# 10XGenomics/lariat

Measured on AMD Instinct MI355X. Metric: read-pairs/sec aligned to hg38 (per-barcode align loop: SMEM seeding + SW + RFA/MAPQ on device); synthetic hg38-scale reference, higher is better.
Workload: dtype u64/i32 (FM-index + integer DP), f64 (RFA scores)

## Files before the change

### lariat_amd/csrc/k_chain_lane.h

```cpp
#pragma once
#include "k_extend2.h"

#ifndef LH_CHAIN_LANE_WAVES
#define LH_CHAIN_LANE_WAVES 2
#endif
#define LH_CHAIN_LANE_MAXC 8
#define CLW(ci_, f_) cl[(((ci_) << 3) + (f_)) * 64 + lane]
#define NIB(x_, i_) ((int)(((x_) >> ((i_) << 2)) & 0xf))
#define NIB_SET(x_, i_, v_) ((x_) = ((x_) & ~(0xfu << ((i_) << 2))) | ((uint32_t)(v_) << ((i_) << 2)))
template <class Lt> __device__ __forceinline__ void dev_introsort_small_nib(int n, uint32_t& a, Lt lt, int32_t* wdp) {
    if (n < 1) return;
    if (n == 2) {
        if (lt(NIB(a, 1), NIB(a, 0))) { int x = NIB(a, 0), y = NIB(a, 1); NIB_SET(a, 0, y); NIB_SET(a, 1, x); }
        return;
    }
    if (n > 1) {
        int t = n - 1, i = 0, j = t, k = i + ((j - i) >> 1) + 1;
        if (lt(NIB(a, k), NIB(a, i))) {
            if (lt(NIB(a, k), NIB(a, j))) k = j;
        } else k = lt(NIB(a, j), NIB(a, i)) ? i : j;
        const int rp = NIB(a, k);
        if (k != t) { int y = NIB(a, t); NIB_SET(a, k, y); NIB_SET(a, t, rp); }
        int wd = 4 * LH_CHAIN_LANE_MAX + 8;
        for (;;) {
            do { ++i; LH_WATCH(wdp, wd, 4, return) } while (lt(NIB(a, i), rp));
            do { --j; LH_WATCH(wdp, wd, 5, return) } while (i <= j && lt(rp, NIB(a, j)));
            if (j <= i) break;
            int x = NIB(a, i), y = NIB(a, j); NIB_SET(a, i, y); NIB_SET(a, j, x);
        }
        { int x = NIB(a, i), y = NIB(a, t); NIB_SET(a, i, y); NIB_SET(a, t, x); }
    }
    for (int i = 1; i < n; ++i)
        for (int j = i; j > 0 && lt(NIB(a, j), NIB(a, j - 1)); --j) { int x = NIB(a, j), y = NIB(a, j - 1); NIB_SET(a, j, y); NIB_SET(a, j - 1, x); }
}
__global__ void __launch_bounds__(64, LH_CHAIN_LANE_WAVES) k_chain_lane(DIndex ix, DOpts o, int n_reads, i64 pool_cap, const DSeed* __restrict__ seeds, const int32_t* __restrict__ s_rid,
                                                    const int32_t* __restrict__ l_rep, DChain* __restrict__ chains, DSeed* __restrict__ cseeds, int32_t* __restrict__ n_chains,
                                                    int32_t* __restrict__ status, int32_t* __restrict__ list, int32_t* __restrict__ list_count, int32_t* __restrict__ srt,
                                                    i64* __restrict__ chain_rmax, DCounters* __restrict__ ctr, ExtArgs A, int fuse,
                                                    int32_t* __restrict__ next_count, int32_t* __restrict__ next_list, int32_t* __restrict__ next_key,
                                                    int32_t* __restrict__ defer_count, int32_t* __restrict__ defer_list) {
    const i64* __restrict__ seq_off = A.seq_off; const i64* __restrict__ seed_off = A.seed_off; int32_t* __restrict__ sdone = A.sdone;
    __shared__ uint32_t cl[LH_CHAIN_LANE_MAXC * 8 * 64];
    const int r = blockIdx.x * blockDim.x + threadIdx.x, lane = LANE();
    int heavy = 0, ext_out = 0, ext_key = 0;
    u64 win = 0, cells = 0;
    int nch_done = 0;
    if (r < n_reads) {
        const i64 base = seed_off[r];
        const int S = (int)(seed_off[r + 1] - base);
        if (seed_off[r + 1] > pool_cap) { n_chains[r] = 0; A.n_regs[r] = 0; atomicOr(&status[r], LH_ST_POOL_OVERFLOW); }
        else if (S > LH_CHAIN_LANE_MAX) heavy = 1;
        else {
            const int len = (int)(seq_off[r + 1] - seq_off[r]);
            const DSeed* sd_ = seeds + base;
            const int32_t* rid_ = s_rid + base;
            int nch = 0;
            uint32_t od = 0;
            u64 smap0 = ~0ull, smap1 = ~0ull;
#define SMAP_SET(s_, v_) { if ((s_) < 16) smap0 = (smap0 & ~(0xfull << ((s_) << 2))) | ((u64)(v_) << ((s_) << 2)); else smap1 = (smap1 & ~(0xfull << (((s_) - 16) << 2))) | ((u64)(v_) << (((s_) - 16) << 2)); }
#define SMAP_GET(s_) ((int)((((s_) < 16 ? smap0 : smap1) >> (((s_) & 15) << 2)) & 0xf))
            DSeed pn; pn.rbeg = 0; pn.qbeg = 0; pn.len = 0;
            int ridn = -1;
            if (S > 0) { pn = sd_[0]; ridn = rid_[0]; }
            for (int s = 0; s < S && !heavy; ++s) {
                const DSeed p = pn;
                const int rid = ridn;
                if (s + 1 < S) { pn = sd_[s + 1]; ridn = rid_[s + 1]; }
                if (rid < 0) continue;
                int to_add = 1, lo = 0;
                for (int k = 0; k < nch; ++k) {
                    const int ci = NIB(od, k);
                    const i64 pos = (i64)((u64)CLW(ci, 0) | (u64)CLW(ci, 1) << 32);
                    if (pos <= p.rbeg) lo = k + 1; else break;
                }
                if (lo > 0) {
                    const int ci = NIB(od, lo - 1);
                    const i64 c_pos = (i64)((u64)CLW(ci, 0) | (u64)CLW(ci, 1) << 32);
                    const uint32_t qp = CLW(ci, 3), ridw = CLW(ci, 4);
                    const i64 c_last_rbeg = c_pos + (int32_t)CLW(ci, 2);
                    const int c_first_qbeg = qp & 0xff, c_last_qbeg = (qp >> 8) & 0xff, c_last_len = (qp >> 16) & 0xff, c_rid = (int)(ridw & 0x3fffffffu);
                    const i64 qend = c_last_qbeg + c_last_len, rend = c_last_rbeg + c_last_len;
                    int res = 0;
                    if (rid != c_rid) res = 0;
                    else if (p.qbeg >= c_first_qbeg && p.qbeg + p.len <= qend && p.rbeg >= c_pos && p.rbeg + p.len <= rend) res = 1;
                    else if ((c_last_rbeg < ix.l_pac || c_pos < ix.l_pac) && p.rbeg >= ix.l_pac) res = 0;
                    else {
                        i64 x = p.qbeg - c_last_qbeg, y = p.rbeg - c_last_rbeg;
                        if (y >= 0 && x - y <= o.w && y - x <= o.w && x - c_last_len < o.max_chain_gap && y - c_last_len < o.max_chain_gap) res = 2;
                    }
                    if (res == 2) {
                        const int rr = (int)(p.rbeg - c_pos);
                        CLW(ci, 2) = (uint32_t)rr;
                        CLW(ci, 3) = (uint32_t)c_first_qbeg | (uint32_t)p.qbeg << 8 | (uint32_t)p.len << 16;
                        uint32_t w5 = CLW(ci, 5), w6 = CLW(ci, 6);
                        int n = w5 & 0xff, wq = (int)(w5 >> 8), endq = w6 & 0xff, wr = (int)(w6 >> 8), endr = (int32_t)CLW(ci, 7);
                        if (p.qbeg >= endq) wq += p.len; else if (p.qbeg + p.len > endq) wq += p.qbeg + p.len - endq;
                        endq = endq > p.qbeg + p.len ? endq : p.qbeg + p.len;
                        if (rr >= endr) wr += p.len; else if (rr + p.len > endr) wr += rr + p.len - endr;
                        endr = endr > rr + p.len ? endr : rr + p.len;
                        CLW(ci, 5) = (uint32_t)(n + 1) | (uint32_t)wq << 8; CLW(ci, 6) = (uint32_t)endq | (uint32_t)wr << 8; CLW(ci, 7) = (uint32_t)endr;
                        SMAP_SET(s, ci)
                    }
                    to_add = (res == 0);
                }
                if (to_add) {
                    if (nch == LH_CHAIN_LANE_MAXC) { heavy = 1; break; }
                    const uint32_t lowm = lo ? (0xffffffffu >> (32 - (lo << 2))) : 0u;
                    od = (od & lowm) | ((uint32_t)nch << (lo << 2)) | ((lo < 7) ? ((od & ~lowm) << 4) : 0u);
                    CLW(nch, 0) = (uint32_t)(u64)p.rbeg; CLW(nch, 1) = (uint32_t)((u64)p.rbeg >> 32); CLW(nch, 2) = 0;
                    CLW(nch, 3) = (uint32_t)p.qbeg | (uint32_t)p.qbeg << 8 | (uint32_t)p.len << 16;
                    CLW(nch, 4) = (uint32_t)rid | ((ix.contig_alt && ix.contig_alt[rid]) ? 1u << 30 : 0u);
                    CLW(nch, 5) = 1u | (uint32_t)p.len << 8; CLW(nch, 6) = (uint32_t)(p.qbeg + p.len) | (uint32_t)p.len << 8; CLW(nch, 7) = (uint32_t)p.len;
                    SMAP_SET(s, nch)
                    nch++;
                }
            }
            if (!heavy) {
            for (int k = 0; k < nch; ++k) {
                const uint32_t w5 = CLW(k, 5), w6 = CLW(k, 6);
                int wq = (int)(w5 >> 8), wr = (int)(w6 >> 8);
                int w = wr < wq ? wr : wq;
                CLW(k, 6) = (uint32_t)(w < 1 << 30 ? w : (1 << 30) - 1);
                CLW(k, 5) = w5 & 0xff;
            }
#define C_W(id_) ((int)CLW(id_, 6))
#define C_BEG(id_) ((int)(CLW(id_, 3) & 0xff))
#define C_END(id_) ((int)(((CLW(id_, 3) >> 8) & 0xff) + ((CLW(id_, 3) >> 16) & 0xff)))
#define C_KEPT(id_) ((int)((CLW(id_, 5) >> 8) & 0xff))
#define C_SET_KEPT(id_, v_) (CLW(id_, 5) = (CLW(id_, 5) & ~0xff00u) | ((uint32_t)(v_) << 8))
#define C_FIRST(id_) ((int)((CLW(id_, 5) >> 16) & 0xff) - 1)
#define C_SET_FIRST(id_, v_) (CLW(id_, 5) = (CLW(id_, 5) & ~0xff0000u) | ((uint32_t)((v_) + 1) << 16))
            uint32_t st = 0;
            int n = 0;
            for (int k = 0; k < nch; ++k) {
                const int id = NIB(od, k);
                if (C_W(id) < o.min_chain_weight) continue;
                NIB_SET(st, n, id); n++;
            }
            if (n > 0) {
                dev_introsort_small_nib(n, st, [&](int x, int y) { return C_W(x) > C_W(y); }, o.wd);
                uint32_t kl = 0;
                int nk = 0;
                C_SET_KEPT(NIB(st, 0), 3);
                NIB_SET(kl, nk, 0); nk++;
                for (int i = 1; i < n; ++i) {
                    int large_ovlp = 0, k;
                    const int idi = NIB(st, i);
                    const int ai_beg = C_BEG(idi), ai_end = C_END(idi), ai_w = C_W(idi), ai_alt = (int)(CLW(idi, 4) >> 30) & 1;
                    for (k = 0; k < nk; ++k) {
                        const int idj = NIB(st, NIB(kl, k));
                        const int aj_beg = C_BEG(idj), aj_end = C_END(idj), aj_w = C_W(idj), aj_alt = (int)(CLW(idj, 4) >> 30) & 1;
                        int b_max = aj_beg > ai_beg ? aj_beg : ai_beg;
                        int e_min = aj_end < ai_end ? aj_end : ai_end;
                        if (e_min > b_max && (!aj_alt || ai_alt)) {
                            int li = ai_end - ai_beg, lj = aj_end - aj_beg;
                            int min_l = li < lj ? li : lj;
                            if (e_min - b_max >= min_l * o.mask_level && min_l < o.max_chain_gap) {
                                large_ovlp = 1;
                                if (C_FIRST(idj) < 0) C_SET_FIRST(idj, i);
                                if (ai_w < aj_w * o.drop_ratio && aj_w - ai_w >= o.min_seed_len << 1) break;
                            }
                        }
                    }
                    if (k == nk) { NIB_SET(kl, nk, i); nk++; C_SET_KEPT(idi, large_ovlp ? 2 : 3); }
                }
                for (int i = 0; i < nk; ++i) {
                    int f = C_FIRST(NIB(st, NIB(kl, i)));
                    if (f >= 0) C_SET_KEPT(NIB(st, f), 1);
                }
                int i, k;
                for (i = k = 0; i < n; ++i) {
                    int kp = C_KEPT(NIB(st, i));
                    if (kp == 0 || kp == 3) continue;
                    if (++k >= o.max_chain_extend) break;
                }
                for (; i < n; ++i)
                    if (C_KEPT(NIB(st, i)) < 3) C_SET_KEPT(NIB(st, i), 0);
            }
            int m = 0, sstart = 0;
            const float frac_rep = (float)l_rep[r] / len;
            for (int i = 0; i < n; ++i) {
                const int id = NIB(st, i);
                const int kp = C_KEPT(id);
                if (kp == 0) { CLW(id, 7) = 0xffffffffu; continue; }
                DChain oc;
                oc.pos = (i64)((u64)CLW(id, 0) | (u64)CLW(id, 1) << 32); oc.rid = (int)(CLW(id, 4) & 0x3fffffffu); oc.n = (int)(CLW(id, 5) & 0xff); oc.seed_start = sstart;
                oc.w = C_W(id); oc.kept = kp; oc.is_alt = (int)(CLW(id, 4) >> 30) & 1;
                oc.frac_rep = frac_rep; oc.pad = id;
                chains[base + m] = oc;
                CLW(id, 7) = (uint32_t)sstart; CLW(id, 2) = 0;
                sstart += oc.n;
                m++;
            }
            for (int k = 0; k < nch; ++k) if (C_W(k) < o.min_chain_weight) CLW(k, 7) = 0xffffffffu;
            for (int s = 0; s < S; ++s) {
                const int id = SMAP_GET(s);
                if (id == 0xf) continue;
                const uint32_t ss = CLW(id, 7);
                if (ss == 0xffffffffu) continue;
                const uint32_t t = CLW(id, 2);
                cseeds[base + ss + t] = sd_[s];
                CLW(id, 2) = t + 1;
            }
            n_chains[r] = m;
#undef SMAP_SET
#undef SMAP_GET
#undef C_W
#undef C_BEG
#undef C_END
#undef C_KEPT
#undef C_SET_KEPT
#undef C_FIRST
#undef C_SET_FIRST
            {
                int l_query = len > LH_MAXLEN ? 0 : len;
                const i64 l_pac = ix.l_pac;
                for (int ci = 0; ci < m; ++ci) {
                    DChain c = chains[base + ci];
                    const DSeed* sd = cseeds + base + c.seed_start;
                    int32_t* so = srt + base + c.seed_start;
                    int32_t* done = sdone + base + c.seed_start;
                    const int n = c.n;
                    if (n == 0) continue;
                    i64 r0 = l_pac << 1, r1 = 0;
                    for (int i = 0; i < n; ++i) {
                        DSeed t = sd[i];
                        i64 b = t.rbeg - (t.qbeg + dev_cal_max_gap(o, t.qbeg));
                        i64 e = t.rbeg + t.len + ((l_query - t.qbeg - t.len) + dev_cal_max_gap(o, l_query - t.qbeg - t.len));
                        r0 = r0 < b ? r0 : b;
                        r1 = r1 > e ? r1 : e;
                    }
                    i64 rmax0 = r0 > 0 ? r0 : 0, rmax1 = r1 < l_pac << 1 ? r1 : l_pac << 1;
                    DSeed s0 = sd[0];
                    if (rmax0 < l_pac && l_pac < rmax1) {
                        if (s0.rbeg < l_pac) rmax1 = l_pac;
                        else rmax0 = l_pac;
                    }
                    dev_fetch_clamp(ix, &rmax0, s0.rbeg, &rmax1);
                    win += (u64)(rmax1 - rmax0);
                    chain_rmax[2 * (base + ci)] = rmax0; chain_rmax[2 * (base + ci) + 1] = rmax1;
                    for (int i = 0; i < n; ++i) {
                        DSeed t = sd[i];
                        int rank = 0;
                        for (int u = 0; u < n; ++u) { DSeed x = sd[u]; rank += (x.len < t.len) || (x.len == t.len && u < i); }
                        so[rank] = i;
                        done[i] = 1;
                    }
                }
                nch_done = m;
            }
            if (fuse) ext_out = ext_control<false>(ix, o, A, r, nullptr, lane, &ext_key, &cells);
            }
        }
    }
    ext_append(ext_out, r, ext_key, lane, next_count, next_list, next_key, defer_count, defer_list);
    if (ctr) {
        unsigned w32 = (unsigned)win;
        u64 wtot = (u64)(uint32_t)wave_sum_i32((int)(w32 >> 16)) << 16;
        wtot += (u64)(uint32_t)wave_sum_i32((int)(w32 & 0xffff));
        int ctot = wave_sum_i32(nch_done);
        if (lane == 0 && (wtot || ctot)) { atomicAdd(&LH_CTR(ctr)->win_bases, wtot); atomicAdd(&LH_CTR(ctr)->n_chain_ext, (u64)ctot); }
    }
    u64 hm = __ballot(heavy);
    if (hm) {
        int basep = 0;
        if (lane == 0) basep = atomicAdd(list_count, (int32_t)__popcll(hm));
        basep = wave_readlane(basep, 0);
        if (heavy) list[basep + lanes_below(hm, lane)] = r;
    }
}
```

### lariat_amd/csrc/k_extend2.h

```cpp
#pragma once
#include "k_extend.h"

#define EH_H(v) ((int)((v) & 0xffffu))
#define EH_E(v) ((int)(((v) >> 16) & 0x1fffu))
#define EH_Q(v) ((int)((v) >> 29))
#define EH_PACK(q, e, h) ((uint32_t)(q) << 29 | (uint32_t)(e) << 16 | (uint32_t)(h))

#define LH_EXT_CIRC_MAX_W 30
__device__ __forceinline__ ExtRes lane_ksw_extend2(const DOpts& o, const uint8_t* q, uint32_t* ehl, int lane, int qoff, int qstep, int qlen, LaneTgt& tg, int tlen, int w,
                                                   int end_bonus, int zdrop, int h0, u64* cells, int circ_mask) {
    const int a_ = o.a, b_ = o.b, o_del = o.o_del, e_del = o.e_del, o_ins = o.o_ins, e_ins = o.e_ins;
    const int oe_del = o_del + e_del, oe_ins = o_ins + e_ins;
#define EHW(j_) ehl[((j_) & circ_mask) * 64 + lane]
    int maxsc = a_ > 0 ? a_ : 0;
    int max_ins = (int)((double)(qlen * maxsc + end_bonus - o_ins) / e_ins + 1.);
    max_ins = max_ins > 1 ? max_ins : 1;
    w = w < max_ins ? w : max_ins;
    int max_del = (int)((double)(qlen * maxsc + end_bonus - o_del) / e_del + 1.);
    max_del = max_del > 1 ? max_del : 1;
    w = w < max_del ? w : max_del;
    int n_mat = 0;
#define EH_MATERIALIZE(upto_)                                                                                \
    for (int lim_ = (upto_) < qlen ? (upto_) : qlen; n_mat <= lim_; ++n_mat) {                               \
        int v_ = n_mat == 0 ? h0 : h0 - oe_ins - (n_mat - 1) * e_ins;                                        \
// ... 96 lines not shown
        if (end > i + w + 1) end = i + w + 1;
        if (end > qlen) end = qlen;
        if (beg == 0) { h1 = h0 - (o_del + e_del * (i + 1)); if (h1 < 0) h1 = 0; }
        else h1 = 0;
        int j, cut = 0;
        if (i == 0) { EH_MAT(1 < qlen ? 1 : qlen, 1) }
        else {
            if (end - beg > 63) { over = 1; break; }
            EH_MAT(end, 0)
        }
        uint32_t p = EHW(beg);
        int fnz = end, lnz = -1;
        for (j = beg; j < end; ++j) {
            if (i == 0 && n_mat <= j + 1) {
                if (j + 1 > 63) { over = 1; break; }
                EH_MAT(j + 1, 1)
            }
            uint32_t pnext = EHW(j + 1);
            int M = EH_H(p), e = EH_E(p);
            int sc = (int32_t)p < 0 ? -1 : ((p ^ tbs) < 0x20000000u ? a_ : -b_);
            const int m_in = M;
            M = M ? M + sc : 0;
            int h = M > e ? M : e;
            h = h > f ? h : f;
            mj = m > h ? mj : j;
            m = m > h ? m : h;
            int t = M - oe_del; t = t > 0 ? t : 0;
            e -= e_del; e = e > t ? e : t;
            EHW(j) = (p & 0xE0000000u) | (uint32_t)e << 16 | (uint32_t)h1;
            if (e | h1) { fnz = fnz < j ? fnz : j; lnz = j; }
            h1 = h;
            t = M - oe_ins; t = t > 0 ? t : 0;
            f -= e_ins; f = f > t ? f : t;
            p = pnext;
            ++ncell;
            if (i == 0 && m_in == 0 && e == 0 && f == 0 && h == 0 && j >= 1) { cut = 1; ++j; break; }
        }
        if (over) break;
        if (cut) {
            h1 = 0;
        } else { uint32_t pe = EHW(end); EHW(end) = EH_PACK(EH_Q(pe), 0, h1); if (h1) lnz = end; }
        if (end == qlen) {
            max_ie = gscore > h1 ? max_ie : i;
            gscore = gscore > h1 ? gscore : h1;
        }
        if (m == 0) break;
        if (m > max) {
            max = m; max_i = i; max_j = mj;
            int d = mj - i; d = d < 0 ? -d : d;
            max_off = max_off > d ? max_off : d;
        } else if (zdrop > 0) {
            if (i - max_i > mj - max_j) {
                if (max - m - ((i - max_i) - (mj - max_j)) * e_del > zdrop) break;
            } else {
                if (max - m - ((mj - max_j) - (i - max_i)) * e_ins > zdrop) break;
            }
        }
        beg = fnz;
        j = lnz >= beg ? lnz : beg - 1;
        end = j + 2 < qlen ? j + 2 : qlen;
    }
#undef EHW
#undef EH_MAT
    if (cells) *cells += ncell;
    *overflow = over;
    ExtRes r;
    r.score = max; r.qle = max_j + 1; r.tle = max_i + 1; r.gtle = max_ie + 1; r.gscore = gscore; r.max_off = max_off;
    return r;
}

#ifndef LH_EXT_ROUNDS
#define LH_EXT_ROUNDS 6
#endif
#define LH_EXT_JOB_BINS 1536
struct ExtSt { int32_t w0, narrow, sc0, w1; };
struct DExtJobs {
    int32_t hist[LH_EXT_JOB_BINS], cursor[LH_EXT_JOB_BINS];
    int32_t count[LH_EXT_ROUNDS + 2];
    int32_t range[2 * (LH_EXT_ROUNDS + 2)];
    int32_t next[LH_EXT_ROUNDS + 2];
    int32_t kinds[3 * (LH_EXT_ROUNDS + 2)];
    int32_t wnext;
    int32_t wave_range[2], heavy_range[2], defer_range[2];
};
__device__ __forceinline__ int lh_ext_job_key(int narrow, int qlen, int h0) {
    const int ql = 31 - (qlen >> 3 < 31 ? qlen >> 3 : 31), hh = 7 - (h0 < 16 ? 0 : h0 < 40 ? (h0 - 16) >> 2 : 6 + (h0 >= 80));
    if (narrow && narrow <= LH_EXT_CIRC_MAX_W) return (LH_EXT_CIRC_MAX_W - narrow) * 32 + ql;
    if (qlen < 64) return 1216 + (31 - (qlen >> 1)) * 8 + hh;
    return 960 + ql * 8 + hh;
}
__global__ void __launch_bounds__(256) k_extj_count(const int32_t* __restrict__ n_jobs, const int32_t* __restrict__ key, DExtJobs* __restrict__ jb) {
    __shared__ int32_t hist[LH_EXT_JOB_BINS];
    const int n = *n_jobs;
    if ((int)blockIdx.x * 1024 >= n) return;
    for (int b = threadIdx.x; b < LH_EXT_JOB_BINS; b += 256) hist[b] = 0;
    __syncthreads();
    for (int blk = blockIdx.x; blk * 1024 < n; blk += gridDim.x)
        for (int u = 0; u < 4; ++u) {
            int i = (blk * 4 + u) * 256 + threadIdx.x;
            if (i < n) atomicAdd(&hist[key[i]], 1);
        }
    __syncthreads();
    for (int b = threadIdx.x; b < LH_EXT_JOB_BINS; b += 256) if (hist[b]) atomicAdd(&jb->hist[b], hist[b]);
}
__global__ void __launch_bounds__(256) k_extj_offsets(DExtJobs* __restrict__ jb, int round, int reuse) {
    __shared__ int32_t part[256];
    const int t = threadIdx.x, per = LH_EXT_JOB_BINS / 256;
    int loc[per], s = 0;
    for (int u = 0; u < per; ++u) { loc[u] = s; s += jb->hist[t * per + u]; }
    part[t] = s;
    __syncthreads();
    for (int d = 1; d < 256; d <<= 1) {
        int o = t >= d ? part[t - d] : 0;
        __syncthreads();
        part[t] += o;
        __syncthreads();
    }
    const int excl = part[t] - s;
    for (int u = 0; u < per; ++u) { const int b = t * per + u, c = jb->hist[b]; if (c) atomicAdd(&jb->kinds[3 * round + (b < 960 ? 0 : b < 1216 ? 1 : 2)], c); }
    for (int u = 0; u < per; ++u) { jb->cursor[t * per + u] = excl + loc[u]; jb->hist[t * per + u] = 0; }
    if (t == 255) {
        jb->range[2 * round] = 0; jb->range[2 * round + 1] = part[255];
        if (reuse >= 0) { jb->count[reuse] = 0; jb->next[round] = 0; jb->count[3] = 0; jb->wnext = 0; }
    }
}
__global__ void __launch_bounds__(256) k_extj_scatter(const int32_t* __restrict__ n_jobs, const int32_t* __restrict__ key, const int32_t* __restrict__ list,
                                                       DExtJobs* __restrict__ jb, int32_t* __restrict__ order) {
    __shared__ int32_t hist[LH_EXT_JOB_BINS], basep[LH_EXT_JOB_BINS];
    const int n = *n_jobs;
    for (int blk = blockIdx.x; blk * 1024 < n; blk += gridDim.x) {
        __syncthreads();
        for (int b = threadIdx.x; b < LH_EXT_JOB_BINS; b += 256) hist[b] = 0;
        __syncthreads();
        int k[4], rank[4];
        for (int u = 0; u < 4; ++u) {
            int i = (blk * 4 + u) * 256 + threadIdx.x;
            k[u] = i < n ? key[i] : -1;
            rank[u] = k[u] >= 0 ? atomicAdd(&hist[k[u]], 1) : 0;
        }
        __syncthreads();
        for (int b = threadIdx.x; b < LH_EXT_JOB_BINS; b += 256) if (hist[b]) basep[b] = atomicAdd(&jb->cursor[b], hist[b]);
        __syncthreads();
        for (int u = 0; u < 4; ++u) {
            int i = (blk * 4 + u) * 256 + threadIdx.x;
            if (k[u] >= 0) order[basep[k[u]] + rank[u]] = list[i];
        }
    }
}

struct ExtArgs {
    const uint8_t* seq; const uint32_t* q4; const i64* seq_off; const i64* seed_off; const DChain* chains; const DSeed* cseeds; const int32_t* n_chains;
    const int32_t* sorder; int32_t* sdone; const i64* chain_rmax; const i64* reg_off; DReg* regs; int32_t* n_regs; ExtSt* est;
    const int32_t* u_read; ExtSt* est_u; int32_t* nreg_u; int32_t* rflag;
};
template <bool DP, bool UNIT = false, bool WAVE = false>
__device__ __forceinline__ int ext_control(const DIndex& ix, const DOpts& o, const ExtArgs& A, const int id, uint32_t* ehl, const int lane, int* key_out, u64* cells_out) {
    const int r = UNIT ? A.u_read[id] : id;
    const uint8_t* seq = A.seq; const uint32_t* q4 = A.q4; const i64* seq_off = A.seq_off; const i64* seed_off = A.seed_off; const DChain* chains = A.chains;
    const DSeed* cseeds = A.cseeds; const int32_t* n_chains = A.n_chains; const int32_t* sorder = A.sorder; int32_t* sdone = A.sdone; const i64* chain_rmax = A.chain_rmax;
    const i64* reg_off = A.reg_off; DReg* regs = A.regs; int32_t* n_regs = A.n_regs; ExtSt* est = A.est;
    int out = 0, key = 0;
    u64 cells = 0;
    {
        const i64 off = seq_off[r];
        int l_query = (int)(seq_off[r + 1] - off);
        if (l_query > LH_MAXLEN) l_query = 0;
// ... 434 lines not shown
```

### lariat_amd/csrc/lh_host.inc

```
#include <math.h>
#include <stdlib.h>
#include <stdio.h>
#include <string.h>

#include <algorithm>
#include <array>
#include <functional>
#include <memory>
#include <mutex>
#include <string>
#include <vector>
#include <map>

#include "../../include/lariat_hip.h"
#include "k_smem4.h"
#include "k_chain_lane.h"
#include "k_chain_cl.h"
#include "k_rfa.h"
#include "k_rescue3.h"
#include "lh_result_cols.h"

#define LH_RFA_FIELDS DInf S; uint8_t* d_slab = nullptr; i64 slab_bytes = 0; int grid_rfa = 0; int32_t* d_bc_next = nullptr; \
    uint8_t* d_slab2 = nullptr; i64 slab2_bytes = 0; int grid_rfa2 = 0; uint8_t* d_slab_mid[2] = {nullptr, nullptr}; i64 slab_mid_bytes[2] = {0, 0}; int grid_rfa_mid[2] = {0, 0}; int grid_rfa_mid_max[2] = {0, 0}; int32_t* d_rfa_ovf_mid = nullptr;  int32_t* d_rfa_ovf = nullptr; int32_t* d_rfa_order = nullptr; int32_t *d_rfa_ovf2 = nullptr, *d_rfa_hp = nullptr, *d_rfa_hr = nullptr; double* d_bc_lmp = nullptr;

// ... 504 lines not shown
        if (tracing) {
            unsigned long long* nul = nullptr;
            HIPCHK(hipMemcpyToSymbolAsync(HIP_SYMBOL(lh_k1_lens), &nul, sizeof nul, 0, hipMemcpyHostToDevice, c->stream));
            unsigned long long hl[2 * 3 * 64];
            HIPCHK(hipMemcpyAsync(hl, d_lens, sizeof hl, hipMemcpyDeviceToHost, c->stream));
            HIPCHK(hipStreamSynchronize(c->stream));
            static const char* const kn[3] = {"ncurr_at_push", "nprev_at_read", "stored_position_read"};
            std::string js = "{";
            for (int ps = 0; ps < 2; ++ps)
                for (int k = 0; k < 3; ++k) {
                    js += std::string(ps || k ? ", " : "") + "\"pass" + std::to_string(ps + 1) + "_" + kn[k] + "\": [";
                    for (int v = 0; v < 64; ++v) js += std::string(v ? ", " : "") + std::to_string(hl[(ps * 3 + k) * 64 + v]);
                    js += "]";
                }
            js += "}";
            fprintf(stderr, "[lh] K1LENS %s\n", js.c_str());
            hipFree(d_lens);
        }
#endif
        T_BEGIN("k_smem4_p3");
        if (o.max_mem_intv > 0 && q4)
            LH_LAUNCH(k_smem_p3_lock, (N + 255) / 256, 256, c->stream, ix4, o, N, q4, (const i64*)c->d_seq_off, c->d_intv, c->d_n_intv, c->d_status, c->d_ctr);
        else if (o.max_mem_intv > 0)
            LH_LAUNCH((k_smem_pass<3, false>), g3, 64, c->stream, ix4, o, N, c->d_seq, c->d_seq_off, c->d_intv, c->d_n_intv, c->d_status, c->d_slab4, c->d_next_read + 2, c->d_ctr, nobig);
        T_END();
        T_BEGIN("k_smem_fin");
        { int rc = k1_big_round(c, o, ix4, N, 0); if (rc) return rc; }
        LH_LAUNCH(k_smem_fin, (N * 16 + 255) / 256, 256, c->stream, o, N, c->d_intv, c->d_n_intv, c->d_seed_cnt, c->d_l_rep, (const int32_t*)c->d_big_slot);
        T_END();
    }
    T_BEGIN("k_scan_seeds");
    { int rc = run_scan(c, N, c->d_seed_cnt, 0, 0, c->d_seed_off); if (rc) return rc; }
    T_END();
    {
        i64 total = 0;
        LH_LAUNCH(k_peek_i64_i32, 1, 1, c->stream, (const i64*)(c->d_seed_off + N), (const int32_t*)(c->d_big_count + 1), c->h_peek);
        HIPCHK(hipStreamSynchronize(c->stream));
        while (c->h_peek[1] > (i64)(c->big_cap - c->big_base)) {
            const i64 asked = c->h_peek[1], old_cap = c->big_cap, new_cap = old_cap + asked + asked / 8 + 16;
            if (new_cap > (1 << 30)) return set_err(LH_E_CAPACITY, "too many reads with more than LH_MAX_INTV SMEM intervals for one batch: split the batch");
            DIntv* slab = nullptr; int32_t* list = nullptr;
            DALLOC(slab, (size_t)new_cap * 2 * LH_BIG_INTV); DALLOC(list, (size_t)new_cap);
            HIPCHK(hipMemcpyAsync(slab, c->d_big_slab, (size_t)old_cap * 2 * LH_BIG_INTV * sizeof(DIntv), hipMemcpyDeviceToDevice, c->stream));
            HIPCHK(hipStreamSynchronize(c->stream));
            hipFree(c->d_big_slab); hipFree(c->d_big_list);
            c->d_big_slab = slab; c->d_big_list = list; c->big_base = (int)old_cap; c->big_cap = (int)new_cap;
            { int rc = k1_big_round(c, o, ix4, N, c->big_base); if (rc) return rc; }
            { int rc = run_scan(c, N, c->d_seed_cnt, 0, 0, c->d_seed_off); if (rc) return rc; }
            LH_LAUNCH(k_peek_i64_i32, 1, 1, c->stream, (const i64*)(c->d_seed_off + N), (const int32_t*)(c->d_big_count + 1), c->h_peek);
            HIPCHK(hipStreamSynchronize(c->stream));
        }
        c->big_base = 0;
        total = c->h_peek[0];
        if (total > c->pool_cap) {
            free_seed_pools(c);
            size_t free_b = 0, total_b = 0;
            HIPCHK(hipMemGetInfo(&free_b, &total_b));
            const double per_seed = sizeof(DSeed) * 2 + 4 * 4 + sizeof(DChainTmp) + sizeof(DChain) + 16 + 2.0 * sizeof(DReg) + 12 + 40;
            const double need = ((double)total * 1.25 + (double)c->cap_reads * LH_RESCUE_SLOTS) * per_seed;
            if (need > (double)free_b - 2e9) {
                c->pool_cap = 0;
                return set_err(LH_E_CAPACITY, "the batch has " + std::to_string(total) + " seeds: their workspace (" + std::to_string((long long)(need / 1e9)) + " GB) does not fit the " +
                                                  std::to_string((long long)(free_b / 1000000000)) + " GB of HBM that are free: split the batch");
            }
            c->pool_cap = total + total / 4;
            c->regpool_cap = c->pool_cap + c->cap_reads * LH_RESCUE_SLOTS;
            int rc = alloc_seed_pools(c);
            if (rc) return rc;
        }
    }
    T_BEGIN("k_seed");
    int g2 = (int)((i64)N * 8 / 256 + 1); if (g2 > 2048) g2 = 2048;
    LH_LAUNCH(k_seed_owner, (N + 255) / 256 < 8192 ? (N + 255) / 256 : 8192, 256, c->stream, N, (const i64*)c->d_seed_off, c->pool_cap, c->d_s_next);
    LH_LAUNCH(k_seed, g2, 256, c->stream, ix, o, N, c->d_seed_off, c->pool_cap, c->d_intv, c->d_n_intv, c->d_seeds, c->d_s_rid, c->d_ctr, (const int32_t*)c->d_s_next, (const int32_t*)c->d_big_slot, (const DIntv*)c->d_big_slab);
    T_END();
    T_BEGIN("k_scan_regs");
    { int rc = run_scan(c, N, c->d_seed_cnt, LH_RESCUE_SLOTS, 0, c->d_reg_off); if (rc) return rc; }
    T_END();
    T_BEGIN("k_chain");
    HIPCHK(hipMemsetAsync(c->d_ext_jobs, 0, sizeof(DExtJobs), c->stream));
    {
        ExtArgs A = ext_args(c);
        const int fuse = (c->flags & LH_F_EXT_WAVE) ? 0 : 1;
        LH_LAUNCH(k_chain_lane, (N + 63) / 64, 64, c->stream, ix, o, N, c->pool_cap, c->d_seeds, c->d_s_rid, c->d_l_rep, c->d_chains, c->d_cseeds, c->d_n_chains, c->d_status,
                  c->d_aln_r, c->d_ext_jobs->wave_range + 1, c->d_srt, c->d_chain_rmax, c->d_ctr, A, fuse, c->d_ext_jobs->count + 1, c->d_ext_jlist, c->d_ext_jkey,
                  c->d_ext_jobs->heavy_range + 1, c->d_ext_heavy);
        const int32_t* wlist = c->d_aln_r;
        const int32_t* wcount = c->d_ext_jobs->wave_range + 1;
        if (!(c->flags & LH_F_CHAIN_WAVE)) {
            int32_t* const fb_count = c->d_aln_count + 3;
            HIPCHK(hipMemsetAsync(fb_count, 0, sizeof(int32_t), c->stream));
#define LH_K3_CL(CAP_, GRID_, LO_, LAST_, ST_)                                                                                                                         \
            LH_LAUNCH((k_chain_cl<CAP_>), N < (GRID_) ? N : (GRID_), 64, ST_, ix, o, (const i64*)c->d_seq_off, (const i64*)c->d_seed_off, c->pool_cap, (const DSeed*)c->d_seeds, \
                      (const int32_t*)c->d_s_rid, (const int32_t*)c->d_l_rep, c->d_chains, c->d_cseeds, c->d_n_chains, c->d_status, wlist, wcount, LO_, LAST_, c->d_aln_ci, fb_count)
            HIPCHK(hipEventRecord(c->ev_fork, c->stream));
            HIPCHK(hipStreamWaitEvent(c->aux[1], c->ev_fork, 0)); HIPCHK(hipStreamWaitEvent(c->aux[2], c->ev_fork, 0));
            LH_K3_CL(LH_CHAIN_CL_CAP_C, 2048, LH_CHAIN_CL_CAP_B, 1, c->aux[2]);
            LH_K3_CL(LH_CHAIN_CL_CAP_B, 8192, LH_CHAIN_CL_CAP_A, 0, c->aux[1]);
            LH_K3_CL(LH_CHAIN_CL_CAP_A, 16384, 0, 0, c->stream);
            HIPCHK(hipEventRecord(c->ev_join[1], c->aux[1])); HIPCHK(hipEventRecord(c->ev_join[2], c->aux[2]));
            HIPCHK(hipStreamWaitEvent(c->stream, c->ev_join[1], 0)); HIPCHK(hipStreamWaitEvent(c->stream, c->ev_join[2], 0));
#undef LH_K3_CL
            wlist = c->d_aln_ci; wcount = fb_count;
#ifdef LH_RFA_PROF
            {
                static const char* const names[8] = {"load + keys", "bitonic sort", "clusters", "cluster walks (lane per cluster)", "order + weights", "introsort", "greedy scan", "emit"};
                unsigned long long h[16];
                HIPCHK(hipStreamSynchronize(c->stream));
                HIPCHK(hipMemcpyFromSymbol(h, HIP_SYMBOL(lh_chain_prof), sizeof h));
                unsigned long long tot = 0;
                for (int i = 0; i < 8; ++i) tot += h[i];
                fprintf(stderr, "[lh] k_chain_cl phases (%llu reads, %.1f k clocks per read):\n", h[15], h[15] ? (double)tot / 1e3 / (double)h[15] : 0.0);
                for (int i = 0; i < 8; ++i) fprintf(stderr, "[lh]   %-36s %6.2f %%\n", names[i], tot ? 100.0 * (double)h[i] / (double)tot : 0.0);
                memset(h, 0, sizeof h);
                HIPCHK(hipMemcpyToSymbol(HIP_SYMBOL(lh_chain_prof), h, sizeof h));
            }
#endif
            if (lh_debug_sync()) {
                int32_t nl = 0, nf = 0;
                if (hipStreamSynchronize(c->stream) == hipSuccess && hipMemcpy(&nl, c->d_ext_jobs->wave_range + 1, 4, hipMemcpyDeviceToHost) == hipSuccess &&
                    hipMemcpy(&nf, fb_count, 4, hipMemcpyDeviceToHost) == hipSuccess)
                    fprintf(stderr, "[lh] K3: %d reads listed for the wave kernels, %d of them left to k_chain by k_chain_cl\n", nl, nf);
            }
        }
        LH_LAUNCH(k_chain, N < 16384 ? N : 16384, 64, c->stream, ix, o, N, c->d_seq_off, c->d_seed_off, c->pool_cap, c->d_seeds, c->d_s_rid, c->d_l_rep, c->d_s_next, c->d_ct,
                  c->d_ord, c->d_srt, c->d_chains, c->d_cseeds, c->d_n_chains, c->d_status, wlist, wcount);
    }
    T_END();
    return LH_OK;
}

static int pipe_align(lh_context* c, const lh_opts* opts) {
    if (!c || !opts) return set_err(LH_E_ARG, "lh_align_resident: null argument");
    if (!c->resident) return set_err(LH_E_ARG, "no batch resident: call lh_batch_upload first");
    if (opts->abi_version != LH_ABI_VERSION) return set_err(LH_E_ARG, "lh_opts.abi_version does not match LH_ABI_VERSION (use lh_opts_init)");
    if (opts->flags & ~(LH_F_NO_SWEEP_FILTER | LH_F_EXT_WAVE | LH_F_EXT_SERIAL | LH_F_CHAIN_WAVE | LH_F_P2_TASKS | LH_F_RESCUE_FULL)) return set_err(LH_E_ARG, "lh_opts.flags: unknown bit set");
    HIPCHK(hipSetDevice(c->idx->device));
    {
        std::vector<void*> fl;
        { std::lock_guard<std::mutex> g(c->slot_mu); fl.swap(c->free_later); }
        for (void* q : fl) hipFree(q);
    }
    DOpts o = to_dopts(opts);
    o.wd = c->d_wd;
    c->flags = opts->flags;
    int t = 0;
    int rc = run_front(c, o, t);
    if (!rc) rc = stage2_run(c, o, t);
    if (rc) {
        for (int i = 0; i < 3; ++i) hipStreamSynchronize(c->aux[i]);
        hipStreamSynchronize(c->stream);
        return rc;
    }
    HIPCHK(hipEventRecord(c->ev[t], c->stream));
    HIPCHK(hipStreamSynchronize(c->stream));
    HIPCHK(hipGetLastError());
    c->n_t = t;
    for (int i = 0; i < t; ++i) HIPCHK(hipEventElapsedTime(&c->tms[i], c->ev[i], c->ev[i + 1]));
    c->ran = true;
    return LH_OK;
}

int lh_last_timings(lh_context* c, int32_t* n, const char* const** names, const float** ms) {
    if (!c) return set_err(LH_E_ARG, "null context");
    if (n) *n = c->n_t;
    if (names) *names = c->tnames;
    if (ms) *ms = c->tms;
    return LH_OK;
}
// ... 87 lines not shown
```

Before: 49.76 million.

## Split lane chaining into a small-capacity pass plus an overflow pass

k_chain_lane is templated on its maximum chain count. It first runs with 4 chain slots, which halves its shared-memory footprint and raises the launch-bounds waves from 2 to 4. Reads that need more than 4 chains are pushed onto a 'more' list and re-run by a grid-strided MAXC=8 pass, so the heavy fallback stays unchanged. The cost is an extra kernel launch and repeated seed scanning for overflow reads. Optional profiling counters sit behind LH_K3_PROF.

```diff
diff --git a/lariat_amd/csrc/k_chain_lane.h b/lariat_amd/csrc/k_chain_lane.h
--- a/lariat_amd/csrc/k_chain_lane.h
+++ b/lariat_amd/csrc/k_chain_lane.h
@@ -1,10 +1,13 @@
 #pragma once
 #include "k_extend2.h"
 
+#define LH_CHAIN_LANE_MAXC 8
+#ifndef LH_CHAIN_LANE_MAXC_SMALL
+#define LH_CHAIN_LANE_MAXC_SMALL 4
+#endif
 #ifndef LH_CHAIN_LANE_WAVES
-#define LH_CHAIN_LANE_WAVES 2
-#endif
-#define LH_CHAIN_LANE_MAXC 8
+#define LH_CHAIN_LANE_WAVES(MAXC_) ((MAXC_) <= 4 ? 4 : 2)
+#endif
 #define CLW(ci_, f_) cl[(((ci_) << 3) + (f_)) * 64 + lane]
 #define NIB(x_, i_) ((int)(((x_) >> ((i_) << 2)) & 0xf))
 #define NIB_SET(x_, i_, v_) ((x_) = ((x_) & ~(0xfu << ((i_) << 2))) | ((uint32_t)(v_) << ((i_) << 2)))
@@ -33,23 +36,37 @@
     for (int i = 1; i < n; ++i)
         for (int j = i; j > 0 && lt(NIB(a, j), NIB(a, j - 1)); --j) { int x = NIB(a, j), y = NIB(a, j - 1); NIB_SET(a, j, y); NIB_SET(a, j - 1, x); }
 }
-__global__ void __launch_bounds__(64, LH_CHAIN_LANE_WAVES) k_chain_lane(DIndex ix, DOpts o, int n_reads, i64 pool_cap, const DSeed* __restrict__ seeds, const int32_t* __restrict__ s_rid,
+#ifdef LH_K3_PROF
+__device__ unsigned long long lh_k3_prof[2][64];
+#endif
+template <int MAXC>
+__global__ void __launch_bounds__(64, LH_CHAIN_LANE_WAVES(MAXC)) k_chain_lane(DIndex ix, DOpts o, int n_reads, i64 pool_cap, const DSeed* __restrict__ seeds, const int32_t* __restrict__ s_rid,
                                                     const int32_t* __restrict__ l_rep, DChain* __restrict__ chains, DSeed* __restrict__ cseeds, int32_t* __restrict__ n_chains,
                                                     int32_t* __restrict__ status, int32_t* __restrict__ list, int32_t* __restrict__ list_count, int32_t* __restrict__ srt,
                                                     i64* __restrict__ chain_rmax, DCounters* __restrict__ ctr, ExtArgs A, int fuse,
                                                     int32_t* __restrict__ next_count, int32_t* __restrict__ next_list, int32_t* __restrict__ next_key,
-                                                    int32_t* __restrict__ defer_count, int32_t* __restrict__ defer_list) {
+                                                    int32_t* __restrict__ defer_count, int32_t* __restrict__ defer_list,
+                                                    const int32_t* __restrict__ in_list, const int32_t* __restrict__ in_count, int32_t* __restrict__ more_list, int32_t* __restrict__ more_count) {
+    static_assert(MAXC >= 1 && MAXC <= 8, "chain ids in the eight nibbles of a register");
     const i64* __restrict__ seq_off = A.seq_off; const i64* __restrict__ seed_off = A.seed_off; int32_t* __restrict__ sdone = A.sdone;
-    __shared__ uint32_t cl[LH_CHAIN_LANE_MAXC * 8 * 64];
-    const int r = blockIdx.x * blockDim.x + threadIdx.x, lane = LANE();
-    int heavy = 0, ext_out = 0, ext_key = 0;
+    __shared__ uint32_t cl[MAXC * 8 * 64];
+    const int lane = LANE();
+    const int n_items = in_list ? *in_count : n_reads;
+    for (int i0 = blockIdx.x * 64; i0 < n_items; i0 += gridDim.x * 64) {
+    const int r = i0 + lane < n_items ? (in_list ? in_list[i0 + lane] : i0 + lane) : n_reads;
+    int heavy = 0, more = 0, ext_out = 0, ext_key = 0;
     u64 win = 0, cells = 0;
     int nch_done = 0;
     if (r < n_reads) {
         const i64 base = seed_off[r];
         const int S = (int)(seed_off[r + 1] - base);
         if (seed_off[r + 1] > pool_cap) { n_chains[r] = 0; A.n_regs[r] = 0; atomicOr(&status[r], LH_ST_POOL_OVERFLOW); }
-        else if (S > LH_CHAIN_LANE_MAX) heavy = 1;
+        else if (S > LH_CHAIN_LANE_MAX) {
+            heavy = 1;
+#ifdef LH_K3_PROF
+            atomicAdd(&lh_k3_prof[1][LH_CHAIN_LANE_MAX + 1], 1ull);
+#endif
+        }
         else {
             const int len = (int)(seq_off[r + 1] - seq_off[r]);
             const DSeed* sd_ = seeds + base;
@@ -104,7 +121,7 @@
                     to_add = (res == 0);
                 }
                 if (to_add) {
-                    if (nch == LH_CHAIN_LANE_MAXC) { heavy = 1; break; }
+                    if (nch == MAXC) { if (more_list) more = 1; else heavy = 1; break; }
                     const uint32_t lowm = lo ? (0xffffffffu >> (32 - (lo << 2))) : 0u;
                     od = (od & lowm) | ((uint32_t)nch << (lo << 2)) | ((lo < 7) ? ((od & ~lowm) << 4) : 0u);
                     CLW(nch, 0) = (uint32_t)(u64)p.rbeg; CLW(nch, 1) = (uint32_t)((u64)p.rbeg >> 32); CLW(nch, 2) = 0;
@@ -115,7 +132,7 @@
                     nch++;
                 }
             }
-            if (!heavy) {
+            if (!heavy && !more) {
             for (int k = 0; k < nch; ++k) {
                 const uint32_t w5 = CLW(k, 5), w6 = CLW(k, 6);
                 int wq = (int)(w5 >> 8), wr = (int)(w6 >> 8);
@@ -251,6 +268,9 @@
             }
             if (fuse) ext_out = ext_control<false>(ix, o, A, r, nullptr, lane, &ext_key, &cells);
             }
+#ifdef LH_K3_PROF
+            if (!more) { atomicAdd(&lh_k3_prof[0][heavy ? MAXC + 1 : nch], 1ull); atomicAdd(&lh_k3_prof[1][S], 1ull); }
+#endif
         }
     }
     ext_append(ext_out, r, ext_key, lane, next_count, next_list, next_key, defer_count, defer_list);
@@ -268,4 +288,12 @@
         basep = wave_readlane(basep, 0);
         if (heavy) list[basep + lanes_below(hm, lane)] = r;
     }
+    u64 mm = __ballot(more);
+    if (mm) {
+        int basep = 0;
+        if (lane == 0) basep = atomicAdd(more_count, (int32_t)__popcll(mm));
+        basep = wave_readlane(basep, 0);
+        if (more) more_list[basep + lanes_below(mm, lane)] = r;
+    }
+    }
 }
diff --git a/lariat_amd/csrc/k_extend2.h b/lariat_amd/csrc/k_extend2.h
--- a/lariat_amd/csrc/k_extend2.h
+++ b/lariat_amd/csrc/k_extend2.h
@@ -202,6 +202,7 @@
     int32_t kinds[3 * (LH_EXT_ROUNDS + 2)];
     int32_t wnext;
     int32_t wave_range[2], heavy_range[2], defer_range[2];
+    int32_t more_range[2];
 };
 __device__ __forceinline__ int lh_ext_job_key(int narrow, int qlen, int h0) {
     const int ql = 31 - (qlen >> 3 < 31 ? qlen >> 3 : 31), hh = 7 - (h0 < 16 ? 0 : h0 < 40 ? (h0 - 16) >> 2 : 6 + (h0 >= 80));
diff --git a/lariat_amd/csrc/lh_host.inc b/lariat_amd/csrc/lh_host.inc
--- a/lariat_amd/csrc/lh_host.inc
+++ b/lariat_amd/csrc/lh_host.inc
@@ -610,9 +610,30 @@
     {
         ExtArgs A = ext_args(c);
         const int fuse = (c->flags & LH_F_EXT_WAVE) ? 0 : 1;
-        LH_LAUNCH(k_chain_lane, (N + 63) / 64, 64, c->stream, ix, o, N, c->pool_cap, c->d_seeds, c->d_s_rid, c->d_l_rep, c->d_chains, c->d_cseeds, c->d_n_chains, c->d_status,
-                  c->d_aln_r, c->d_ext_jobs->wave_range + 1, c->d_srt, c->d_chain_rmax, c->d_ctr, A, fuse, c->d_ext_jobs->count + 1, c->d_ext_jlist, c->d_ext_jkey,
-                  c->d_ext_jobs->heavy_range + 1, c->d_ext_heavy);
+#define LH_K3_LANE(MAXC_, GRID_, IN_, IN_COUNT_, MORE_, MORE_COUNT_)                                                                                                  \
+        LH_LAUNCH((k_chain_lane<MAXC_>), GRID_, 64, c->stream, ix, o, N, c->pool_cap, c->d_seeds, c->d_s_rid, c->d_l_rep, c->d_chains, c->d_cseeds, c->d_n_chains, c->d_status, \
+                  c->d_aln_r, c->d_ext_jobs->wave_range + 1, c->d_srt, c->d_chain_rmax, c->d_ctr, A, fuse, c->d_ext_jobs->count + 1, c->d_ext_jlist, c->d_ext_jkey,       \
+                  c->d_ext_jobs->heavy_range + 1, c->d_ext_heavy, IN_, IN_COUNT_, MORE_, MORE_COUNT_)
+        if (LH_CHAIN_LANE_MAXC_SMALL < LH_CHAIN_LANE_MAXC) {
+            LH_K3_LANE(LH_CHAIN_LANE_MAXC_SMALL, (N + 63) / 64, (const int32_t*)nullptr, (const int32_t*)nullptr, c->d_aln_ci, c->d_ext_jobs->more_range + 1);
+            LH_K3_LANE(LH_CHAIN_LANE_MAXC, (N + 63) / 64 < 2048 ? (N + 63) / 64 : 2048, (const int32_t*)c->d_aln_ci, (const int32_t*)(c->d_ext_jobs->more_range + 1), (int32_t*)nullptr, (int32_t*)nullptr);
+        } else
+            LH_K3_LANE(LH_CHAIN_LANE_MAXC, (N + 63) / 64, (const int32_t*)nullptr, (const int32_t*)nullptr, (int32_t*)nullptr, (int32_t*)nullptr);
+#undef LH_K3_LANE
+#ifdef LH_K3_PROF
+        {
+            unsigned long long h[2][64];
+            HIPCHK(hipStreamSynchronize(c->stream));
+            HIPCHK(hipMemcpyFromSymbol(h, HIP_SYMBOL(lh_k3_prof), sizeof h));
+            std::string js = "{\"chains\": [";
+            for (int i = 0; i <= LH_CHAIN_LANE_MAXC + 1; ++i) js += std::string(i ? ", " : "") + std::to_string(h[0][i]);
+            js += "], \"seeds\": [";
+            for (int i = 0; i <= LH_CHAIN_LANE_MAX + 1; ++i) js += std::string(i ? ", " : "") + std::to_string(h[1][i]);
+            fprintf(stderr, "[lh] K3PROF %s]}\n", js.c_str());
+            memset(h, 0, sizeof h);
+            HIPCHK(hipMemcpyToSymbol(HIP_SYMBOL(lh_k3_prof), h, sizeof h));
+        }
+#endif
         const int32_t* wlist = c->d_aln_r;
         const int32_t* wcount = c->d_ext_jobs->wave_range + 1;
         if (!(c->flags & LH_F_CHAIN_WAVE)) {
```

Measured after the change: 49.92 million, median of 4. Within noise of the previous version (+0.3%).
